# mahbodnr/ViT-CIFAR

Hardware: NVIDIA B200
Metric: train images/s (fwd+bwd+Adam) (higher is better)
Workload: dtype bf16

## Files before the change

### include/vitb200.h

```cpp
#ifndef VITB200_H_
#define VITB200_H_

#include <stddef.h>
#include <stdint.h>

#ifdef __cplusplus
extern "C" {
#endif

#define VITB_F32 0
#define VITB_BF16 1

#define VITB_ABI_VERSION 1

int vitb_version(void);
const char* vitb_last_error(void);
unsigned long long vitb_launch_count(void);
int vitb_device_supported(void);

int vitb_set_l2_persisting_window(void* base, size_t bytes, size_t carve_out_bytes);

int vitb_cast_f32_to_bf16(const float* src, void* dst, int64_t n, void* stream);

size_t vitb_patch_embed_fwd_ws_bytes(int B, int S, int P, int H, int dt);
// ... 17 lines not shown
#define VITB_GEMM_GELU 1
#define VITB_GEMM_OUT_F32 2
int vitb_gemm_bias_act_fwd(const void* a, const void* w_act, const float* bias, const void* residual,
                           void* c, void* preact, int M, int N, int K, int flags, int dt, void* stream);
int vitb_gemm_dgrad(const void* dy, const void* w_act, const void* z, void* dx, int M, int N, int K,
                    int flags, int dt, void* stream);
#define VITB_GEMM_DY_F32 4
size_t vitb_gemm_wgrad_ws_bytes(int M, int N, int K, int dt);
int vitb_gemm_wgrad_dbias(const void* dy, const void* x, float* dw, float* dbias, void* ws,
                          size_t ws_bytes, int M, int N, int K, int flags, int dt, void* stream);

int vitb_attn_fwd(const void* qkv, void* o, float* lse, float* attn_map, int B, int T, int heads,
                  int d, float scale, int dt, void* stream);
int vitb_attn_bwd(const void* qkv, const void* o, const void* d_o, const float* lse, void* dqkv, int B,
                  int T, int heads, int d, float scale, int dt, void* stream);

size_t vitb_colsum_ws_bytes(int rows, int cols);
int vitb_gelu_bwd_colsum(const void* dy, const void* z, void* dz, float* colsum, void* ws,
                         size_t ws_bytes, int rows, int cols, int dt, void* stream);
int vitb_colsum(const void* x, float* colsum, void* ws, size_t ws_bytes, int rows, int cols, int dt,
                void* stream);

int vitb_augment_crop_flip_normalize(const uint8_t* img_u8, const int32_t* dx, const int32_t* dy, const uint8_t* flip,
                                     const float* mean3, const float* std3, float* out, int B, int S, int pad, void* stream);

int vitb_augment_autoaugment(const uint8_t* img_u8, const int32_t* dx, const int32_t* dy, const uint8_t* flip, const int32_t* code,
                             const int32_t* op_ids, const double* mags, int n_sub, const float* mean3, const float* std3,
                             float* out, int B, int S, int pad, void* stream);

int vitb_augment_crop_flip_normalize_gather(const uint8_t* data_u8, const int64_t* labels_src, int N, const int32_t* idx,
// ... 82 lines not shown
```

### vit-cifar_b200/_lib.py

```python
from __future__ import annotations

import ctypes as C
import os
import threading

HERE = os.path.dirname(os.path.abspath(__file__))
LIB_PATH = os.environ.get("VITB_LIB_PATH") or os.path.join(HERE, "libvitb200.so")

F32 = 0
BF16 = 1

GEMM_GELU = 1
GEMM_OUT_F32 = 2
GEMM_DY_F32 = 4

ABI_VERSION = 1

_p = C.c_void_p
_i = C.c_int
_i64 = C.c_int64
_f = C.c_float
_sz = C.c_size_t

class DropoutDesc(C.Structure):
# ... 10 lines not shown
    "vitb_set_l2_persisting_window": (_i, [_p, _sz, _sz]),
    "vitb_cast_f32_to_bf16": (_i, [_p, _p, _i64, _p]),
    "vitb_patch_embed_fwd_ws_bytes": (_sz, [_i, _i, _i, _i, _i]),
    "vitb_patch_embed_fwd": (_i, [_p, _p, _p, _p, _p, _p, _p, _p, _p, _sz, _i, _i, _i, _i, _i, _i, _p]),
    "vitb_patch_embed_bwd_ws_bytes": (_sz, [_i, _i, _i, _i, _i]),
    "vitb_patch_embed_bwd": (_i, [_p, _p, _p, _p, _p, _p, _p, _p, _sz, _i, _i, _i, _i, _i, _i, _p]),
    "vitb_layernorm_fwd": (_i, [_p, _i64, _p, _p, _p, _p, _p, _i, _i, _f, _i, _p]),
    "vitb_layernorm_bwd_ws_bytes": (_sz, [_i, _i]),
    "vitb_layernorm_bwd": (_i, [_p, _p, _i64, _p, _p, _p, _p, _p, _i64, _p, _p, _p, _p, _sz, _i, _i, _i, _p]),
    "vitb_gemm_bias_act_fwd": (_i, [_p, _p, _p, _p, _p, _p, _i, _i, _i, _i, _i, _p]),
    "vitb_gemm_dgrad": (_i, [_p, _p, _p, _p, _i, _i, _i, _i, _i, _p]),
    "vitb_gemm_wgrad_ws_bytes": (_sz, [_i, _i, _i, _i]),
    "vitb_gemm_wgrad_dbias": (_i, [_p, _p, _p, _p, _p, _sz, _i, _i, _i, _i, _i, _p]),
    "vitb_attn_fwd": (_i, [_p, _p, _p, _p, _i, _i, _i, _i, _f, _i, _p]),
    "vitb_attn_bwd": (_i, [_p, _p, _p, _p, _p, _i, _i, _i, _i, _f, _i, _p]),
    "vitb_colsum_ws_bytes": (_sz, [_i, _i]),
    "vitb_gelu_bwd_colsum": (_i, [_p, _p, _p, _p, _p, _sz, _i, _i, _i, _p]),
    "vitb_colsum": (_i, [_p, _p, _p, _sz, _i, _i, _i, _p]),
    "vitb_pool_fwd": (_i, [_p, _p, _i, _i, _i, _i, _i, _p]),
    "vitb_pool_bwd": (_i, [_p, _p, _i, _i, _i, _i, _i, _p]),
    "vitb_augment_crop_flip_normalize": (_i, [_p, _p, _p, _p, _p, _p, _p, _i, _i, _i, _p]),
    "vitb_augment_autoaugment": (_i, [_p, _p, _p, _p, _p, _p, _p, _i, _p, _p, _p, _i, _i, _i, _p]),
    "vitb_augment_crop_flip_normalize_gather": (_i, [_p, _p, _i, _p, _p, _p, _p, _p, _p, _p, _p, _i, _i, _i, _p]),
    "vitb_augment_autoaugment_gather": (_i, [_p, _p, _i, _p, _p, _p, _p, _p, _p, _p, _i, _p, _p, _p, _p, _i, _i, _i, _p]),
    "vitb_batch_mix": (_i, [_p, _p, _p, _i, _i, _i, _i, C.c_double, _i, _i, _i, _i, _p]),
    "vitb_dropout_threshold": (C.c_uint32, [_f]),
    "vitb_dropout": (_i, [_p, _p, _p, _i64, _f, C.c_uint64, C.c_uint32, C.c_uint32, _p, _i, _p]),
    "vitb_ls_ce_fwd_bwd": (_i, [_p, _p, _p, _p, _i, _i, _f, _f, _p]),
    "vitb_ls_ce_mix_fwd_bwd": (_i, [_p, _p, _p, _f, _p, _p, _p, _i, _i, _f, _f, _p]),
    "vitb_ls_ce_batch_fwd_bwd": (_i, [_p, _p, _p, _f, _p, _p, _p, _p, _i, _i, _f, _f, _p]),
# ... 60 lines not shown
```

### vit-cifar_b200/csrc/attention.cu

```cuda
#include <cuda.h>

#include "common.cuh"
#include "gemm_internal.h"

namespace vitb {

__device__ __forceinline__ void ldsm_x4(uint32_t (&r)[4], const void* p) {
  const uint32_t a = (uint32_t)__cvta_generic_to_shared(p);
  asm volatile("ldmatrix.sync.aligned.m8n8.x4.shared.b16 {%0,%1,%2,%3}, [%4];" : "=r"(r[0]), "=r"(r[1]), "=r"(r[2]), "=r"(r[3]) : "r"(a));
}
__device__ __forceinline__ void ldsm_x4_t(uint32_t (&r)[4], const void* p) {
  const uint32_t a = (uint32_t)__cvta_generic_to_shared(p);
  asm volatile("ldmatrix.sync.aligned.m8n8.x4.trans.shared.b16 {%0,%1,%2,%3}, [%4];" : "=r"(r[0]), "=r"(r[1]), "=r"(r[2]), "=r"(r[3]) : "r"(a));
}
__device__ __forceinline__ void stsm_x4(void* p, uint32_t r0, uint32_t r1, uint32_t r2, uint32_t r3) {
  const uint32_t a = (uint32_t)__cvta_generic_to_shared(p);
  asm volatile("stmatrix.sync.aligned.m8n8.x4.shared.b16 [%0], {%1,%2,%3,%4};" ::"r"(a), "r"(r0), "r"(r1), "r"(r2), "r"(r3) : "memory");
}
__device__ __forceinline__ void mma_bf16(float (&d)[4], const uint32_t (&a)[4], uint32_t b0, uint32_t b1) {
  asm volatile(
      "mma.sync.aligned.m16n8k16.row.col.f32.bf16.bf16.f32 {%0,%1,%2,%3}, {%4,%5,%6,%7}, {%8,%9}, {%0,%1,%2,%3};"
      : "+f"(d[0]), "+f"(d[1]), "+f"(d[2]), "+f"(d[3])
      : "r"(a[0]), "r"(a[1]), "r"(a[2]), "r"(a[3]), "r"(b0), "r"(b1));
}
// ... 410 lines not shown

  stage_rows16<D>(dq, sQ, 16 * warp, lane);
  stage_rows16<D>(dk, sK, 16 * warp, lane);
  stage_rows16<D>(dv, sV, 16 * warp, lane);
  fence_async_smem();
  __syncthreads();
  if (tid == 0) {
    tma_store_3d(&m_dqkv, sQ, h * D, 0, b);
    tma_store_3d(&m_dqkv, sK, Hd + h * D, 0, b);
    tma_store_3d(&m_dqkv, sV, 2 * Hd + h * D, 0, b);
    tma_store_commit();
    tma_store_wait_read();
  }
}

__global__ void __launch_bounds__(128)
    attn_fwd_f32_kernel(const float* __restrict__ qkv, float* __restrict__ o, float* __restrict__ lse, float* __restrict__ attn_map,
                        int T, int heads, int D, float scale) {
  pdl_trigger();
  pdl_wait();
  extern __shared__ __align__(16) uint8_t smem_attn[];
  float* sQ = reinterpret_cast<float*>(smem_attn);
  float* sK = sQ + T * D;
  float* sV = sK + T * D;
  float* sS = sV + T * D;
  const int b = blockIdx.x / heads, h = blockIdx.x % heads, Hd = heads * D;
  const int tid = threadIdx.x, nthr = blockDim.x;
  const float* base = qkv + (int64_t)b * T * 3 * Hd + h * D;
  for (int i = tid; i < T * D; i += nthr) {
    const int r = i / D, c = i % D;
// ... 127 lines not shown
    configured = true;
  }
  const int Hd = heads * D;
  CUtensorMap m_qkv, m_o, m_do, m_dqkv;
  if (head_tile_map<D, NT16>(&m_qkv, qkv, 3 * Hd, T, B)) return -1;
  if (head_tile_map<D, NT16>(&m_o, o, Hd, T, B)) return -1;
  if (head_tile_map<D, NT16>(&m_do, d_o, Hd, T, B)) return -1;
  if (head_tile_map<D, NT16>(&m_dqkv, dqkv, 3 * Hd, T, B)) return -1;
  int per_sm = 1;
  VITB_CUDA_OK(cudaOccupancyMaxActiveBlocksPerMultiprocessor(&per_sm, kern, 32 * NT16, smem));
  VITB_LAUNCH((kern), B * heads, 32 * NT16, smem, st, m_qkv, m_o, m_do, m_dqkv, lse, T, heads, scale, kNumSMs * (per_sm > 0 ? per_sm : 1));
  VITB_LAUNCH_OK();
  return 0;
}

#define VITB_ATTN_DISPATCH(FN, ...)                                                   \
  do {                                                                                \
    const int nt = (T + 15) / 16;                                                     \
    if (d == 32) {                                                                    \
      if (nt <= 1) return FN<32, 1>(__VA_ARGS__);                                     \
      if (nt <= 2) return FN<32, 2>(__VA_ARGS__);                                     \
      if (nt <= 4) return FN<32, 4>(__VA_ARGS__);                                     \
      if (nt <= 5) return FN<32, 5>(__VA_ARGS__);                                     \
      return FN<32, 8>(__VA_ARGS__);                                                  \
    } else {                                                                          \
      if (nt <= 1) return FN<64, 1>(__VA_ARGS__);                                     \
      if (nt <= 2) return FN<64, 2>(__VA_ARGS__);                                     \
      if (nt <= 4) return FN<64, 4>(__VA_ARGS__);                                     \
      if (nt <= 5) return FN<64, 5>(__VA_ARGS__);                                     \
      return FN<64, 8>(__VA_ARGS__);                                                  \
// ... 28 lines not shown
int vitb_attn_bwd(const void* qkv, const void* o, const void* d_o, const float* lse, void* dqkv, int B, int T, int heads, int d, float scale,
                  int dt, void* stream) {
  VITB_REQUIRE(qkv && o && d_o && lse && dqkv, "attn_bwd: null pointer");
  VITB_REQUIRE(B > 0 && T > 0 && T <= 128 && heads > 0 && (d == 32 || d == 64), "attn_bwd: unsupported shape B=%d T=%d heads=%d d=%d (T<=128, d in {32,64})", B, T, heads, d);
  cudaStream_t st = (cudaStream_t)stream;
  if (dt == VITB_BF16) {
    VITB_ATTN_DISPATCH(launch_bwd_bf16, qkv, o, d_o, lse, dqkv, B, T, heads, scale, st);
  }
  const size_t smem = ((size_t)4 * T * d + (size_t)2 * T * T) * sizeof(float);
  if (set_dyn_smem((const void*)attn_bwd_f32_kernel, smem)) return -1;
  VITB_LAUNCH((attn_bwd_f32_kernel), B * heads, 128, smem, st, (const float*)qkv, (const float*)d_o, lse, (float*)dqkv, T, heads, d, scale);
  VITB_LAUNCH_OK();
  return 0;
}

}
```

### vit-cifar_b200/engine.py

```python
from __future__ import annotations

import os
from typing import Dict, Optional, Tuple

import torch

from . import functional as Fn
from . import ops
from .layers import act_dtype
from .optim import adam_hyper, sgd_hyper
from .parallel import allreduce_bucket
from .params import LayerViews
from .vit import ViT


class TrainEngine:
    def __init__(self, model: ViT, batch_size: int, smoothing: float = 0.1, lr: float = 1e-3, betas=(0.9, 0.999),
                 eps: float = 1e-8, weight_decay: float = 5e-5, process_group=None, use_graph: bool = True,
                 overlap_comm: bool = False, mixed_targets: bool = False, optimizer: str = "adam", momentum: Optional[float] = None,
                 metrics: bool = False):
        ops.require_device()
        if optimizer not in ("adam", "sgd"):
            raise NotImplementedError(f"Unknown optimizer: {optimizer}")
        self.optimizer = optimizer
# ... 52 lines not shown
                peers, err = None, ValueError("at most 8 ranks of one node and a flat buffer that is a multiple of 4 elements")
            else:
                peers, err = exchange_peer_pointers(dict(g=self.G, p=self.P, c=self.C if self.C is not self.P else None, flags=flags), self.pg)
            ok = torch.tensor([0 if peers is None else 1], device=self.dev)
            dist.all_reduce(ok, op=dist.ReduceOp.MIN, group=self.pg)
            if int(ok.item()) == 1:
                self._fused_dp = dict(peers, flags_t=flags, sync=sync, rank=dist.get_rank(self.pg))
            else:
                import warnings
                warnings.warn(f"fused data-parallel step unavailable ({err}); using one NCCL all-reduce + the Adam kernel")
                self._dp_mode = mode = "single"

        H, M = model.hidden, model.mlp_hidden
        self.dm = Fn.Dims(B=self.B, T=model.num_tokens, H=H, heads=model.head, M=M, use_mlp=model.encoder_mlp)
        self.dm.check()
        mk = lambda buf, i: LayerViews(L, buf, f"enc.{i}.", H, M, model.encoder_mlp)
        self.lp = [mk(self.P, i) for i in range(model.num_layers)]
        self.lc = [mk(self.C, i) for i in range(model.num_layers)]
        self.lg = [mk(self.G, i) for i in range(model.num_layers)]
        v = L.view
        self.has_cls = model.is_cls_token
        self.stem_p = (v(self.P, "emb.weight"), v(self.P, "emb.bias"),
                       v(self.P, "cls_token").view(-1) if self.has_cls else None, v(self.P, "pos_emb").view(model.num_tokens, H))
        self.stem_g = (v(self.G, "emb.weight"), v(self.G, "emb.bias"),
                       v(self.G, "cls_token").view(-1) if self.has_cls else None, v(self.G, "pos_emb").view(model.num_tokens, H))
        self.head_p = (v(self.P, "fc.0.weight"), v(self.P, "fc.0.bias"), v(self.C, "fc.1.weight"), v(self.P, "fc.1.bias"))
        self.head_g = (v(self.G, "fc.0.weight"), v(self.G, "fc.0.bias"), v(self.G, "fc.1.weight"), v(self.G, "fc.1.bias"))
        self.buckets = model.bucket_bounds()

        S = model.img_size
# ... 43 lines not shown
        self._main_stream = None
        env = os.environ.get("VITB_FLUSH_PER_LAYER")
        self._flush_per_layer = (env != "0") if env is not None else (model.hidden * max(model.hidden, model.mlp_hidden) <= 384 * 1536)
        self._opt_per_layer = self._flush_per_layer and self.world == 1 and os.environ.get("VITB_OPT_PER_LAYER", "1") != "0"
        self._opt_done_from = 0
        if ws_mode >= 1:
            if ws_mode >= 2:
                self._main_stream = torch.cuda.Stream(device=self.dev, priority=-1)
            self._side = Fn.SideStream(torch.cuda.Stream(device=self.dev))

    def _alloc(self, scope: str):
        def alloc(name: str, shape: tuple, dtype: torch.dtype) -> torch.Tensor:
            key = f"{scope}.{name}"
            t = self._bufs.get(key)
            if t is None:
                t = (torch.zeros if name == "dxL" else torch.empty)(shape, dtype=dtype, device=self.dev)
                self._bufs[key] = t
            return t
        return alloc

    def _arena_bytes(self) -> int:
        from . import _lib
        lib, dm, m = _lib.load(), self.dm, self.model
        rows, H, M = dm.rows, dm.H, dm.M
        ln = int(lib.vitb_layernorm_bwd_ws_bytes(rows, H))
        pair = lambda N, K: max(ops.wgrad_ws_bytes(rows, N, K), ops.bwd_fused_ws_bytes(rows, N, K))
        per_layer = pair(H, H) + ops.wgrad_ws_bytes(rows, 3 * H, H) + ln
        if dm.use_mlp:
            per_layer += pair(H, M) + pair(M, H) + ln + int(lib.vitb_colsum_ws_bytes(rows, H))
        per_layer += 8 * 256
        return m.num_layers * per_layer + int(lib.vitb_layernorm_bwd_ws_bytes(self.B, H)) + (1 << 20)

    def activation_bytes(self) -> int:
        return sum(t.numel() * t.element_size() for t in self._bufs.values())

    def _allreduce(self, bucket: Tuple[int, int], last: bool = False) -> None:
        if self.world == 1:
            return
        if self._dp_mode in ("none", "fused"):
            return
        if self.overlap_comm:
            allreduce_bucket(self.G, bucket, self.pg, self._comm_stream)
        elif last:
            allreduce_bucket(self.G, (0, self.n), self.pg, None)

    def _body(self) -> None:
        m, dm = self.model, self.dm
        B, T, H, Cn = self.B, m.num_tokens, m.hidden, m.num_classes
        emb_w, emb_b, cls, pos = self.stem_p
        emb_w_c = self.store.layout.view(self.C, "emb.weight") if self.C is not self.P else None
        x, words = Fn.stem_fwd(self.img, emb_w, emb_w_c, emb_b, cls, pos, m.patch, self.act, self._alloc("stem"))
        saved = []
        for i in range(m.num_layers):
            x, sv = Fn.encoder_fwd(x, self.lc[i], self.lp[i], dm, self._alloc(f"l{i}"), drop=self.drops[i] if self.drops else None)
            saved.append(sv)
        ln_w, ln_b, fc_w_c, fc_b = self.head_p
        self.logits, hsaved = Fn.head_fwd(x, ln_w, ln_b, fc_w_c, fc_b, B, T, H, Cn, m.is_cls_token, self._alloc("head"))
        n_valid_dev = self.hyper_dev.view(torch.int32)[11:12]
        if self.mixed_targets:
            ops.ls_ce(self.logits, self.labels, self.loss, self.dlogits, self.smoothing, 1.0, labels_b=self.labels_b, lam_dev=self.hyper_dev[9:10],
                      n_valid_dev=n_valid_dev, ws=self._ls_ws)
        else:
            ops.ls_ce(self.logits, self.labels, self.loss, self.dlogits, self.smoothing, 1.0, n_valid_dev=n_valid_dev, ws=self._ls_ws)
        if self.metrics:
            ops.eval_metrics(self.logits, self.labels, self._record[:3], self._record_ws, self.smoothing, n_valid_dev=n_valid_dev)
            ops.train_loss_accumulate(self.loss, self._record[3:], self.B, n_valid_dev=n_valid_dev)

        self._opt_done_from = self.n
        self._backward(hsaved, saved, words)
        n = self.n
        if self._fused_dp is not None:
            f = self._fused_dp
# ... 17 lines not shown
        ln_w, ln_b, fc_w_c, fc_b = self.head_p
        if self._main_stream is not None:
            outer = torch.cuda.current_stream()
            self._main_stream.wait_stream(outer)
            with torch.cuda.stream(self._main_stream):
                self._backward_kernels(hsaved, saved, words, B, T, H, Cn, ln_w, fc_w_c)
            outer.wait_stream(self._main_stream)
        else:
            self._backward_kernels(hsaved, saved, words, B, T, H, Cn, ln_w, fc_w_c)

    def _backward_kernels(self, hsaved, saved, words, B, T, H, Cn, ln_w, fc_w_c) -> None:
        m, dm, side = self.model, self.dm, self._side
        if self._defer:
            ops.defer_begin(self._arena)
        g_ln_w, g_ln_b, g_fc_w, g_fc_b = self.head_g
        dx = Fn.head_bwd(self.dlogits, hsaved, ln_w, fc_w_c, g_ln_w, g_ln_b, g_fc_w, g_fc_b, B, T, H, Cn, m.is_cls_token, self.act,
                         self._alloc("headb"), dx_prezeroed=True, side=side)
        self._allreduce(self.buckets[-1])
        done = {}
        fuse_below = (Fn.ln_gelu_fused() and dm.use_mlp and self.act == torch.bfloat16 and (not self.drops or Fn._drop_fused(dm.rows)))
        dz2_in = None
        for i in reversed(range(m.num_layers)):
            if side is not None and (i + 2) in done:
                torch.cuda.current_stream().wait_event(done[i + 2])
            below = None
            if fuse_below and i > 0:
                dz2_b = self._alloc(f"bwd_dz2_{(i - 1) % 3}")("dz2", (dm.rows, dm.H), self.act)
                below = (saved[i - 1][4][6], dz2_b, self.lg[i - 1].b2, self.drops[i - 1] if self.drops else None)
            dx = Fn.encoder_bwd(dx, saved[i], self.lc[i], self.lp[i], self.lg[i], dm, self._bwd_alloc(i),
                                drop=self.drops[i] if self.drops else None, side=side, dz2_in=dz2_in, below=below)
            dz2_in = below[1] if below is not None else None
            if side is not None:
                if self._defer and self._flush_per_layer:
                    side.run(ops.defer_flush_partial)
                    if self._opt_per_layer:
                        lo = self.buckets[1 + i][0]
                        hi = self._opt_done_from
                        side.run(lambda lo=lo, hi=hi: self._optimizer_slice(lo, hi))
                        self._opt_done_from = lo
                done[i] = side.done_event()
            self._allreduce(self.buckets[1 + i])
        g_emb_w, g_emb_b, g_cls, g_pos = self.stem_g
        Fn.stem_bwd(self.img, words, dx, g_emb_w, g_emb_b, g_cls, g_pos, m.patch)
        if side is not None:
            side.join()
# ... 182 lines not shown
```

### vit-cifar_b200/functional.py

```python
from __future__ import annotations

import os
from dataclasses import dataclass
from typing import Callable, Optional

import torch

from . import ops
from .params import LayerViews

Alloc = Callable[[str, tuple, torch.dtype], torch.Tensor]


def default_alloc(device: torch.device) -> Alloc:
    def alloc(name: str, shape: tuple, dtype: torch.dtype) -> torch.Tensor:
        return torch.empty(shape, dtype=dtype, device=device)
    return alloc


@dataclass
class Dims:
    B: int
    T: int
    H: int
# ... 70 lines not shown
        return ops.drop_desc(self.p, self.seed, site, self.step, self.step_dev)


DROP_FUSED_MIN_ROWS = 16384


def _drop_fused(rows: int = 1 << 30) -> bool:
    v = os.environ.get("VITB_DROP_FUSED", "auto")
    if v in ("0", "1"):
        return v == "1"
    return rows >= DROP_FUSED_MIN_ROWS


def ln_gelu_fused() -> bool:
    return os.environ.get("VITB_LN_GELU_FUSED", "0") != "0"


def mhsa_fwd(x: torch.Tensor, c: LayerViews, p: LayerViews, dm: Dims, alloc: Alloc, residual: Optional[torch.Tensor],
             attn_map: Optional[torch.Tensor] = None, drop: Optional[Drop] = None):
    rows, H, act = dm.rows, dm.H, x.dtype
    qkv = alloc("qkv", (rows, 3 * H), act)
    ops.gemm_fwd(x, c.wqkv, p.bqkv, None, qkv, None, rows, 3 * H, H)
    o = alloc("o", (rows, H), act)
    lse = alloc("lse", (dm.B, dm.heads, dm.T), torch.float32)
    ops.attn_fwd(qkv, o, lse, attn_map, dm.B, dm.T, dm.heads, dm.d, dm.scale)
    y = alloc("x1", (rows, H), act)
    if drop is None or _drop_fused(rows):
        ops.gemm_fwd(o, c.wo, p.bo, residual, y, None, rows, H, H, drop=drop.desc(0) if drop is not None else None)
    else:
        ops.gemm_fwd(o, c.wo, p.bo, None, y, None, rows, H, H)
# ... 93 lines not shown
            _wgrad(side, dz1, x1n, g.w1, None if b1_done else g.b1, rows, M, H)
            ops.gemm_dgrad(dz1, c.w1, None, dx1n, rows, M, H)
        dx1 = alloc("dx1", (rows, H), act)
        if fused_drop:
            dya = alloc("dao", (rows, H), act)
            ops.layernorm_bwd_fused(dx1n, x1, H, p.ln2_w, mean2, rstd2, dout, dx1, H, g.ln2_w, g.ln2_b, None, dya, g.bo, rows, H,
                                    drop=drop.desc(0))
            bo_done = True
        else:
            bo_done = drop is None
            ops.layernorm_bwd(dx1n, x1, H, p.ln2_w, mean2, rstd2, dout, dx1, H, g.ln2_w, g.ln2_b, g.bo if bo_done else None, rows, H)
    else:
        dx1 = dout
        bo_done = False
    dxn = mhsa_bwd(dx1, att_saved, c, g, dm, alloc, bo_done=bo_done, drop=drop, side=side, dy_masked=dya)
    dx = alloc("dx", (rows, H), act)
    if below is not None:
        z2_b, dz2_b, g_b2_b, drop_b = below
        ops.layernorm_bwd_fused(dxn, x, H, p.ln1_w, mean1, rstd1, dx1, dx, H, g.ln1_w, g.ln1_b, z2_b, dz2_b, g_b2_b, rows, H,
                                drop=drop_b.desc(2) if drop_b is not None else None)
    else:
        ops.layernorm_bwd(dxn, x, H, p.ln1_w, mean1, rstd1, dx1, dx, H, g.ln1_w, g.ln1_b, None, rows, H)
    return dx


def stem_fwd(img: torch.Tensor, emb_w, emb_w_c, emb_b, cls, pos, P: int, act: torch.dtype, alloc: Alloc):
    B, _, S, _ = img.shape
    has_cls = cls is not None
    T = P * P + (1 if has_cls else 0)
    H, K = emb_w.shape
    x0 = alloc("x0", (B * T, H), act)
    words = alloc("words", (B * P * P, K), act) if (act == torch.bfloat16 and emb_w_c is not None) else None
    ops.patch_embed_fwd(img, emb_w, emb_w_c if words is not None else None, emb_b, cls, pos, x0, words, P, has_cls)
    return x0, words


def stem_bwd(img: torch.Tensor, words, dx0: torch.Tensor, g_emb_w, g_emb_b, g_cls, g_pos, P: int) -> None:
    ops.patch_embed_bwd(img, words, dx0, g_emb_w, g_emb_b, g_cls, g_pos, P, g_cls is not None)
# ... 34 lines not shown
```

### vit-cifar_b200/ops.py

```python
from __future__ import annotations

import ctypes as C
from typing import Optional

import torch

from . import _lib
from ._lib import BF16, F32, GEMM_DY_F32, GEMM_GELU, GEMM_OUT_F32, check

_DT = {torch.float32: F32, torch.bfloat16: BF16}


def dt_of(t: torch.Tensor) -> int:
    try:
        return _DT[t.dtype]
    except KeyError:
        raise TypeError(f"activation dtype must be float32 or bfloat16, got {t.dtype}") from None


def _ptr(t: Optional[torch.Tensor]) -> Optional[int]:
    if t is None:
        return None
    if not t.is_cuda:
        raise _lib.VitbError("libvitb200 kernels take CUDA tensors only (no CPU fallback)")
# ... 134 lines not shown
    lib = _lib.load()
    dt = dt_of(x)
    nb = lib.vitb_gemm_bwd_fused_ws_bytes(M, N, K, dt)
    ws = workspace(max(int(nb), 256), x.device)
    check(lib.vitb_gemm_bwd_fused(_ptr(dy), _ptr(x), _ptr(w_act), _ptr(z), _ptr(dx), _ptr(dw), _ptr(dx_colsum), _ptr(ws), ws.numel(), M, N, K, dt,
                                  _stream()), "gemm_bwd_fused")


def attn_fwd(qkv, o, lse, attn_map, B: int, T: int, heads: int, d: int, scale: float) -> None:
    check(_lib.load().vitb_attn_fwd(_ptr(qkv), _ptr(o), _ptr(lse), _ptr(attn_map), B, T, heads, d, scale, dt_of(qkv), _stream()), "attn_fwd")


def attn_bwd(qkv, o, d_o, lse, dqkv, B: int, T: int, heads: int, d: int, scale: float) -> None:
    check(_lib.load().vitb_attn_bwd(_ptr(qkv), _ptr(o), _ptr(d_o), _ptr(lse), _ptr(dqkv), B, T, heads, d, scale, dt_of(qkv), _stream()),
          "attn_bwd")


def gelu_bwd_colsum(dy, z, dz, colsum, rows: int, cols: int, drop=None) -> None:
    lib = _lib.load()
    ws = workspace(lib.vitb_colsum_ws_bytes(rows, cols), dy.device)
    check(lib.vitb_gelu_bwd_colsum_drop(_ptr(dy), _ptr(z), _ptr(dz), _ptr(colsum), _ptr(ws), ws.numel(), rows, cols, dt_of(dy), _dref(drop),
                                        _stream()), "gelu_bwd_colsum")


def colsum(x, out, rows: int, cols: int) -> None:
    lib = _lib.load()
    ws = workspace(lib.vitb_colsum_ws_bytes(rows, cols), x.device)
    check(lib.vitb_colsum(_ptr(x), _ptr(out), _ptr(ws), ws.numel(), rows, cols, dt_of(x), _stream()), "colsum")


# ... 249 lines not shown
```

Baseline: 171,700.

## Compute only the CLS token in the last encoder layer

When the model classifies from the CLS token, the last encoder layer now computes attention only for the CLS query, and runs the output projection and MLP only on B rows instead of B*T rows. New single-warp forward and backward attention kernels handle the one-query case, and the backward scatters the CLS residual gradient back into a zeroed full-row buffer. This removes the per-token work in the last layer whose outputs the head never reads. In exchange it adds new kernels and a separate code path that is used only for bf16, zero dropout and batch size of at least 32.

```diff
diff --git a/include/vitb200.h b/include/vitb200.h
--- a/include/vitb200.h
+++ b/include/vitb200.h
@@ -55,6 +55,10 @@
                   int d, float scale, int dt, void* stream);
 int vitb_attn_bwd(const void* qkv, const void* o, const void* d_o, const float* lse, void* dqkv, int B,
                   int T, int heads, int d, float scale, int dt, void* stream);
+int vitb_attn_cls_fwd(const void* qkv, void* o_c, float* lse_c, int B, int T, int heads, int d, float scale, int dt,
+                      void* stream);
+int vitb_attn_cls_bwd(const void* qkv, const void* o_c, const void* do_c, const float* lse_c, void* dqkv, int B, int T,
+                      int heads, int d, float scale, int dt, void* stream);
 
 size_t vitb_colsum_ws_bytes(int rows, int cols);
 int vitb_gelu_bwd_colsum(const void* dy, const void* z, void* dz, float* colsum, void* ws,
diff --git a/vit-cifar_b200/_lib.py b/vit-cifar_b200/_lib.py
--- a/vit-cifar_b200/_lib.py
+++ b/vit-cifar_b200/_lib.py
@@ -48,6 +48,8 @@
     "vitb_gemm_wgrad_dbias": (_i, [_p, _p, _p, _p, _p, _sz, _i, _i, _i, _i, _i, _p]),
     "vitb_attn_fwd": (_i, [_p, _p, _p, _p, _i, _i, _i, _i, _f, _i, _p]),
     "vitb_attn_bwd": (_i, [_p, _p, _p, _p, _p, _i, _i, _i, _i, _f, _i, _p]),
+    "vitb_attn_cls_fwd": (_i, [_p, _p, _p, _i, _i, _i, _i, _f, _i, _p]),
+    "vitb_attn_cls_bwd": (_i, [_p, _p, _p, _p, _p, _i, _i, _i, _i, _f, _i, _p]),
     "vitb_colsum_ws_bytes": (_sz, [_i, _i]),
     "vitb_gelu_bwd_colsum": (_i, [_p, _p, _p, _p, _p, _sz, _i, _i, _i, _p]),
     "vitb_colsum": (_i, [_p, _p, _p, _sz, _i, _i, _i, _p]),
diff --git a/vit-cifar_b200/csrc/attention.cu b/vit-cifar_b200/csrc/attention.cu
--- a/vit-cifar_b200/csrc/attention.cu
+++ b/vit-cifar_b200/csrc/attention.cu
@@ -448,6 +448,233 @@
   }
 }
 
+template <int D, int NT16>
+__global__ void __launch_bounds__(32)
+    attn_cls_fwd_bf16_kernel(const __grid_constant__ CUtensorMap m_q, const __grid_constant__ CUtensorMap m_qkv, bf16* __restrict__ o,
+                             float* __restrict__ lse, int T, int heads, float scale, int pf_dist) {
+  constexpr int TP = 16 * NT16;
+  constexpr uint32_t TILE_B = TP * D * 2, ROWS_B = 16 * D * 2;
+  extern __shared__ uint8_t smem_attn_raw[];
+  const uint32_t sbase = (smem_u32(smem_attn_raw) + 1023u) & ~1023u;
+  const uint32_t sQ = sbase, sK = sQ + ROWS_B, sV = sK + TILE_B, bar = sV + TILE_B;
+  const int b = blockIdx.x / heads, h = blockIdx.x % heads, Hd = heads * D;
+  const int lane = threadIdx.x;
+  pdl_trigger();
+  if (lane == 0) {
+    mbar_init(bar, 1);
+    asm volatile("fence.mbarrier_init.release.cluster;" ::: "memory");
+  }
+  __syncthreads();
+  pdl_wait();
+  if (lane == 0) {
+    mbar_arrive_expect_tx(bar, ROWS_B + 2 * TILE_B);
+    tma_load_3d(sQ, &m_q, bar, h * D, 0, b);
+    tma_load_3d(sK, &m_qkv, bar, Hd + h * D, 0, b);
+    tma_load_3d(sV, &m_qkv, bar, 2 * Hd + h * D, 0, b);
+    const int nxt = (int)blockIdx.x + pf_dist;
+    if (nxt < (int)gridDim.x) {
+      const int nb = nxt / heads, nh = nxt % heads;
+      tma_prefetch_3d(&m_qkv, Hd + nh * D, 0, nb);
+      tma_prefetch_3d(&m_qkv, 2 * Hd + nh * D, 0, nb);
+    }
+  }
+  const int g = lane >> 2, t = lane & 3;
+  const float sl2 = scale * kLog2e;
+  const KeyMask km = make_key_mask(T, lane);
+  const LaneAddr<D> la(lane);
+  mbar_wait(bar, 0);
+
+  float s[2 * NT16][4];
+  qk_tile<D, NT16>(s, sQ, sK, 0, la, km);
+  float m0 = -INFINITY, m1 = -INFINITY;
+#pragma unroll
+  for (int j = 0; j < 2 * NT16; ++j) {
+    m0 = fmaxf(m0, fmaxf(s[j][0], s[j][1]));
+    m1 = fmaxf(m1, fmaxf(s[j][2], s[j][3]));
+  }
+  m0 = quad_max(m0);
+  m1 = quad_max(m1);
+  const float ms0 = m0 * sl2, ms1 = m1 * sl2;
+  float sum0 = 0.f, sum1 = 0.f;
+#pragma unroll
+  for (int j = 0; j < 2 * NT16; ++j) {
+    s[j][0] = ex2_fast(fmaf(s[j][0], sl2, -ms0));
+    s[j][1] = ex2_fast(fmaf(s[j][1], sl2, -ms0));
+    s[j][2] = ex2_fast(fmaf(s[j][2], sl2, -ms1));
+    s[j][3] = ex2_fast(fmaf(s[j][3], sl2, -ms1));
+    sum0 += s[j][0] + s[j][1];
+    sum1 += s[j][2] + s[j][3];
+  }
+  sum0 = quad_sum(sum0);
+  const float inv0 = 1.0f / sum0;
+  float acc[D / 8][4];
+#pragma unroll
+  for (int jn = 0; jn < D / 8; ++jn) acc[jn][0] = acc[jn][1] = acc[jn][2] = acc[jn][3] = 0.f;
+  pv_tile<D, NT16>(acc, s, sV, la);
+  if (g == 0) {
+    if (t == 0) lse[(int64_t)b * heads + h] = m0 * scale + logf(sum0);
+    bf16* orow = o + (int64_t)b * Hd + h * D;
+#pragma unroll
+    for (int jn = 0; jn < D / 8; ++jn)
+      *reinterpret_cast<uint32_t*>(orow + 8 * jn + 2 * t) = pack_bf16x2(acc[jn][0] * inv0, acc[jn][1] * inv0);
+  }
+}
+
+template <int D, int NT16>
+__global__ void __launch_bounds__(32)
+    attn_cls_bwd_bf16_kernel(const __grid_constant__ CUtensorMap m_q, const __grid_constant__ CUtensorMap m_qkv, const __grid_constant__ CUtensorMap m_o,
+                             const __grid_constant__ CUtensorMap m_do, const __grid_constant__ CUtensorMap m_dqkv, const float* __restrict__ lse,
+                             int T, int heads, float scale, int pf_dist) {
+  constexpr int TP = 16 * NT16, LP = TP + 8, CH = D / 8;
+  constexpr uint32_t TILE_B = TP * D * 2, ROWS_B = 16 * D * 2;
+  extern __shared__ uint8_t smem_attn_raw[];
+  const uint32_t sbase = (smem_u32(smem_attn_raw) + 1023u) & ~1023u;
+  uint8_t* gen = smem_attn_raw + (sbase - smem_u32(smem_attn_raw));
+  const uint32_t sQ = sbase, sK = sQ + TILE_B, sV = sK + TILE_B, sdO = sV + TILE_B, sO = sdO + ROWS_B;
+  bf16* sP = reinterpret_cast<bf16*>(gen + 3 * TILE_B + 2 * ROWS_B);
+  bf16* sdS = sP + 16 * LP;
+  float* sD = reinterpret_cast<float*>(sdS + 16 * LP);
+  const uint32_t bar = smem_u32(sD + 16);
+  const int b = blockIdx.x / heads, h = blockIdx.x % heads, Hd = heads * D;
+  const int lane = threadIdx.x;
+  pdl_trigger();
+  pdl_wait();
+  if (lane == 0) {
+    mbar_init(bar, 1);
+    asm volatile("fence.mbarrier_init.release.cluster;" ::: "memory");
+    mbar_arrive_expect_tx(bar, 3 * TILE_B + 2 * ROWS_B);
+    tma_load_3d(sQ, &m_q, bar, h * D, 0, b);
+    tma_load_3d(sK, &m_qkv, bar, Hd + h * D, 0, b);
+    tma_load_3d(sV, &m_qkv, bar, 2 * Hd + h * D, 0, b);
+    tma_load_3d(sdO, &m_do, bar, h * D, 0, b);
+    tma_load_3d(sO, &m_o, bar, h * D, 0, b);
+    const int nxt = (int)blockIdx.x + pf_dist;
+    if (nxt < (int)gridDim.x) {
+      const int nb = nxt / heads, nh = nxt % heads;
+      tma_prefetch_3d(&m_qkv, Hd + nh * D, 0, nb);
+      tma_prefetch_3d(&m_qkv, 2 * Hd + nh * D, 0, nb);
+    }
+  }
+  const int g = lane >> 2;
+  const float l0 = g == 0 ? lse[(int64_t)b * heads + h] * kLog2e : 0.f, l1 = 0.f;
+  __syncthreads();
+  mbar_wait(bar, 0);
+  for (int idx = lane; idx < 16 * CH; idx += 32) {
+    const int r = idx / CH, c = idx % CH;
+    uint32_t a0, a1, a2, a3, q0, q1, q2, q3;
+    const uint32_t off = tile_off<D>(r, c);
+    asm volatile("ld.shared.v4.b32 {%0, %1, %2, %3}, [%4];" : "=r"(a0), "=r"(a1), "=r"(a2), "=r"(a3) : "r"(sdO + off));
+    asm volatile("ld.shared.v4.b32 {%0, %1, %2, %3}, [%4];" : "=r"(q0), "=r"(q1), "=r"(q2), "=r"(q3) : "r"(sO + off));
+    const float2 x0 = unpack_bf16x2(a0), x1 = unpack_bf16x2(a1), x2 = unpack_bf16x2(a2), x3 = unpack_bf16x2(a3);
+    const float2 y0 = unpack_bf16x2(q0), y1 = unpack_bf16x2(q1), y2 = unpack_bf16x2(q2), y3 = unpack_bf16x2(q3);
+    float v = (x0.x * y0.x + x0.y * y0.y) + (x1.x * y1.x + x1.y * y1.y) + (x2.x * y2.x + x2.y * y2.y) + (x3.x * y3.x + x3.y * y3.y);
+#pragma unroll
+    for (int off2 = CH / 2; off2 > 0; off2 >>= 1) v += __shfl_xor_sync(0xffffffffu, v, off2);
+    if (c == 0) sD[r] = v;
+  }
+  __syncwarp();
+
+  const float sl2 = scale * kLog2e;
+  const float d0 = sD[g], d1 = sD[g + 8];
+  const KeyMask km = make_key_mask(T, lane);
+  const LaneAddr<D> la(lane);
+  uint32_t aq[D / 16][4], ado[D / 16][4];
+#pragma unroll
+  for (int kk = 0; kk < D / 16; ++kk) {
+    ldsm_x4_s(aq[kk], sQ + la.a(0, kk));
+    ldsm_x4_s(ado[kk], sdO + la.a(0, kk));
+  }
+  float dq[D / 8][4];
+#pragma unroll
+  for (int jn = 0; jn < D / 8; ++jn) dq[jn][0] = dq[jn][1] = dq[jn][2] = dq[jn][3] = 0.f;
+#pragma unroll
+  for (int jc = 0; jc < NT16; ++jc) {
+    float s[2][4], dp[2][4];
+#pragma unroll
+    for (int u = 0; u < 2; ++u) {
+      const int j = 2 * jc + u;
+      s[u][0] = s[u][1] = s[u][2] = s[u][3] = 0.f;
+      dp[u][0] = dp[u][1] = dp[u][2] = dp[u][3] = 0.f;
+      if (j < km.nfull || (j == km.nfull && km.rem != 0)) {
+#pragma unroll
+        for (int k2 = 0; k2 < D / 32; ++k2) {
+          uint32_t bk[4], bv[4];
+          ldsm_x4_s(bk, sK + la.b(8 * j, k2));
+          ldsm_x4_s(bv, sV + la.b(8 * j, k2));
+          mma_bf16(s[u], aq[2 * k2], bk[0], bk[1]);
+          mma_bf16(s[u], aq[2 * k2 + 1], bk[2], bk[3]);
+          mma_bf16(dp[u], ado[2 * k2], bv[0], bv[1]);
+          mma_bf16(dp[u], ado[2 * k2 + 1], bv[2], bv[3]);
+        }
+        if (j == km.nfull) {
+          s[u][0] += km.pm0; s[u][2] += km.pm0;
+          s[u][1] += km.pm1; s[u][3] += km.pm1;
+        }
+        s[u][0] = ex2_fast(fmaf(s[u][0], sl2, -l0));
+        s[u][1] = ex2_fast(fmaf(s[u][1], sl2, -l0));
+        s[u][2] = ex2_fast(fmaf(s[u][2], sl2, -l1));
+        s[u][3] = ex2_fast(fmaf(s[u][3], sl2, -l1));
+        dp[u][0] = s[u][0] * (dp[u][0] - d0) * scale;
+        dp[u][1] = s[u][1] * (dp[u][1] - d0) * scale;
+        dp[u][2] = s[u][2] * (dp[u][2] - d1) * scale;
+        dp[u][3] = s[u][3] * (dp[u][3] - d1) * scale;
+      }
+    }
+    uint32_t pa[4], da[4];
+    pa[0] = pack_bf16x2(s[0][0], s[0][1]); pa[1] = pack_bf16x2(s[0][2], s[0][3]);
+    pa[2] = pack_bf16x2(s[1][0], s[1][1]); pa[3] = pack_bf16x2(s[1][2], s[1][3]);
+    da[0] = pack_bf16x2(dp[0][0], dp[0][1]); da[1] = pack_bf16x2(dp[0][2], dp[0][3]);
+    da[2] = pack_bf16x2(dp[1][0], dp[1][1]); da[3] = pack_bf16x2(dp[1][2], dp[1][3]);
+    const int srow = ((lane >> 3) & 1) * 8 + (lane & 7), scol = 16 * jc + (lane >> 4) * 8;
+    stsm_x4(sP + srow * LP + scol, pa[0], pa[1], pa[2], pa[3]);
+    stsm_x4(sdS + srow * LP + scol, da[0], da[1], da[2], da[3]);
+#pragma unroll
+    for (int jp = 0; jp < D / 16; ++jp) {
+      uint32_t bb[4];
+      ldsm_x4_t_s(bb, sK + la.t(16 * jc, jp));
+      mma_bf16(dq[2 * jp], da, bb[0], bb[1]);
+      mma_bf16(dq[2 * jp + 1], da, bb[2], bb[3]);
+    }
+  }
+  __syncwarp();
+
+  for (int kt = 0; kt < NT16; ++kt) {
+    float dv[D / 8][4], dk[D / 8][4];
+#pragma unroll
+    for (int jn = 0; jn < D / 8; ++jn) {
+      dv[jn][0] = dv[jn][1] = dv[jn][2] = dv[jn][3] = 0.f;
+      dk[jn][0] = dk[jn][1] = dk[jn][2] = dk[jn][3] = 0.f;
+    }
+    const int arow = ((lane & 7) + ((lane >> 4) & 1) * 8) * LP + 16 * kt + ((lane >> 3) & 1) * 8;
+    uint32_t ap[4], as[4];
+    ldsm_x4_t(ap, sP + arow);
+    ldsm_x4_t(as, sdS + arow);
+#pragma unroll
+    for (int jp = 0; jp < D / 16; ++jp) {
+      uint32_t bo[4], bq[4];
+      ldsm_x4_t_s(bo, sdO + la.t(0, jp));
+      ldsm_x4_t_s(bq, sQ + la.t(0, jp));
+      mma_bf16(dv[2 * jp], ap, bo[0], bo[1]);
+      mma_bf16(dv[2 * jp + 1], ap, bo[2], bo[3]);
+      mma_bf16(dk[2 * jp], as, bq[0], bq[1]);
+      mma_bf16(dk[2 * jp + 1], as, bq[2], bq[3]);
+    }
+    stage_rows16<D>(dk, sK, 16 * kt, lane);
+    stage_rows16<D>(dv, sV, 16 * kt, lane);
+  }
+  __syncwarp();
+  stage_rows16<D>(dq, sQ, 0, lane);
+  fence_async_smem();
+  __syncwarp();
+  if (lane == 0) {
+    tma_store_3d(&m_dqkv, sQ, h * D, 0, b);
+    tma_store_3d(&m_dqkv, sK, Hd + h * D, 0, b);
+    tma_store_3d(&m_dqkv, sV, 2 * Hd + h * D, 0, b);
+    tma_store_commit();
+    tma_store_wait_read();
+  }
+}
+
 __global__ void __launch_bounds__(128)
     attn_fwd_f32_kernel(const float* __restrict__ qkv, float* __restrict__ o, float* __restrict__ lse, float* __restrict__ attn_map,
                         int T, int heads, int D, float scale) {
@@ -605,6 +832,55 @@
   return 0;
 }
 
+template <int D>
+static int row0_map(CUtensorMap* map, const void* ptr, int cols, int T, int B, int box_rows) {
+  return make_tma_map_3d_bf16(map, ptr, (uint64_t)cols, 1, (uint64_t)B, (uint64_t)cols * 2, (uint64_t)T * cols * 2, D, box_rows, 1, D == 32 ? 64 : 128);
+}
+
+template <int D, int NT16>
+static int launch_cls_fwd_bf16(const void* qkv, void* o, float* lse, int B, int T, int heads, float scale, cudaStream_t st) {
+  constexpr int TP = 16 * NT16;
+  constexpr size_t smem = (size_t)16 * D * 2 + (size_t)2 * TP * D * 2 + 16 + 1024;
+  auto kern = attn_cls_fwd_bf16_kernel<D, NT16>;
+  static int per_sm = 0;
+  if (per_sm == 0) {
+    VITB_CUDA_OK(cudaFuncSetAttribute(kern, cudaFuncAttributeMaxDynamicSharedMemorySize, (int)smem));
+    VITB_CUDA_OK(cudaOccupancyMaxActiveBlocksPerMultiprocessor(&per_sm, kern, 32, smem));
+    if (per_sm < 1) per_sm = 1;
+  }
+  const int Hd = heads * D;
+  CUtensorMap m_q, m_qkv;
+  if (row0_map<D>(&m_q, qkv, 3 * Hd, T, B, 16)) return -1;
+  if (head_tile_map<D, NT16>(&m_qkv, qkv, 3 * Hd, T, B)) return -1;
+  VITB_LAUNCH((kern), B * heads, 32, smem, st, m_q, m_qkv, (bf16*)o, lse, T, heads, scale, kNumSMs * per_sm);
+  VITB_LAUNCH_OK();
+  return 0;
+}
+
+template <int D, int NT16>
+static int launch_cls_bwd_bf16(const void* qkv, const void* o, const void* d_o, const float* lse, void* dqkv, int B, int T, int heads, float scale,
+                               cudaStream_t st) {
+  constexpr int TP = 16 * NT16, LP = TP + 8;
+  constexpr size_t smem = (size_t)3 * TP * D * 2 + (size_t)2 * 16 * D * 2 + (size_t)2 * 16 * LP * 2 + 16 * sizeof(float) + 16 + 1024;
+  auto kern = attn_cls_bwd_bf16_kernel<D, NT16>;
+  static int per_sm = 0;
+  if (per_sm == 0) {
+    VITB_CUDA_OK(cudaFuncSetAttribute(kern, cudaFuncAttributeMaxDynamicSharedMemorySize, (int)smem));
+    VITB_CUDA_OK(cudaOccupancyMaxActiveBlocksPerMultiprocessor(&per_sm, kern, 32, smem));
+    if (per_sm < 1) per_sm = 1;
+  }
+  const int Hd = heads * D;
+  CUtensorMap m_q, m_qkv, m_o, m_do, m_dqkv;
+  if (row0_map<D>(&m_q, qkv, 3 * Hd, T, B, TP)) return -1;
+  if (head_tile_map<D, NT16>(&m_qkv, qkv, 3 * Hd, T, B)) return -1;
+  if (row0_map<D>(&m_o, o, Hd, 1, B, 16)) return -1;
+  if (row0_map<D>(&m_do, d_o, Hd, 1, B, 16)) return -1;
+  if (head_tile_map<D, NT16>(&m_dqkv, dqkv, 3 * Hd, T, B)) return -1;
+  VITB_LAUNCH((kern), B * heads, 32, smem, st, m_q, m_qkv, m_o, m_do, m_dqkv, lse, T, heads, scale, kNumSMs * per_sm);
+  VITB_LAUNCH_OK();
+  return 0;
+}
+
 #define VITB_ATTN_DISPATCH(FN, ...)                                                   \
   do {                                                                                \
     const int nt = (T + 15) / 16;                                                     \
@@ -663,4 +939,21 @@
   return 0;
 }
 
-}
+int vitb_attn_cls_fwd(const void* qkv, void* o_c, float* lse_c, int B, int T, int heads, int d, float scale, int dt, void* stream) {
+  VITB_REQUIRE(qkv && o_c && lse_c, "attn_cls_fwd: null pointer");
+  VITB_REQUIRE(dt == VITB_BF16, "attn_cls_fwd: bf16 only (dt=%d)", dt);
+  VITB_REQUIRE(B > 0 && T > 0 && T <= 128 && heads > 0 && (d == 32 || d == 64), "attn_cls_fwd: unsupported shape B=%d T=%d heads=%d d=%d (T<=128, d in {32,64})", B, T, heads, d);
+  cudaStream_t st = (cudaStream_t)stream;
+  VITB_ATTN_DISPATCH(launch_cls_fwd_bf16, qkv, o_c, lse_c, B, T, heads, scale, st);
+}
+
+int vitb_attn_cls_bwd(const void* qkv, const void* o_c, const void* do_c, const float* lse_c, void* dqkv, int B, int T, int heads, int d,
+                      float scale, int dt, void* stream) {
+  VITB_REQUIRE(qkv && o_c && do_c && lse_c && dqkv, "attn_cls_bwd: null pointer");
+  VITB_REQUIRE(dt == VITB_BF16, "attn_cls_bwd: bf16 only (dt=%d)", dt);
+  VITB_REQUIRE(B > 0 && T > 0 && T <= 128 && heads > 0 && (d == 32 || d == 64), "attn_cls_bwd: unsupported shape B=%d T=%d heads=%d d=%d (T<=128, d in {32,64})", B, T, heads, d);
+  cudaStream_t st = (cudaStream_t)stream;
+  VITB_ATTN_DISPATCH(launch_cls_bwd_bf16, qkv, o_c, do_c, lse_c, dqkv, B, T, heads, scale, st);
+}
+
+}
diff --git a/vit-cifar_b200/engine.py b/vit-cifar_b200/engine.py
--- a/vit-cifar_b200/engine.py
+++ b/vit-cifar_b200/engine.py
@@ -90,6 +90,8 @@
         H, M = model.hidden, model.mlp_hidden
         self.dm = Fn.Dims(B=self.B, T=model.num_tokens, H=H, heads=model.head, M=M, use_mlp=model.encoder_mlp)
         self.dm.check()
+        self._cls_tail = Fn.cls_tail(model.is_cls_token, self.act, model.p_drop, self.B)
+        self._head_T = 1 if self._cls_tail else model.num_tokens
         mk = lambda buf, i: LayerViews(L, buf, f"enc.{i}.", H, M, model.encoder_mlp)
         self.lp = [mk(self.P, i) for i in range(model.num_layers)]
         self.lc = [mk(self.C, i) for i in range(model.num_layers)]
@@ -163,7 +165,7 @@
             key = f"{scope}.{name}"
             t = self._bufs.get(key)
             if t is None:
-                t = (torch.zeros if name == "dxL" else torch.empty)(shape, dtype=dtype, device=self.dev)
+                t = (torch.zeros if name in ("dxL", "dx1_rows") else torch.empty)(shape, dtype=dtype, device=self.dev)
                 self._bufs[key] = t
             return t
         return alloc
@@ -172,13 +174,16 @@
         from . import _lib
         lib, dm, m = _lib.load(), self.dm, self.model
         rows, H, M = dm.rows, dm.H, dm.M
-        ln = int(lib.vitb_layernorm_bwd_ws_bytes(rows, H))
-        pair = lambda N, K: max(ops.wgrad_ws_bytes(rows, N, K), ops.bwd_fused_ws_bytes(rows, N, K))
-        per_layer = pair(H, H) + ops.wgrad_ws_bytes(rows, 3 * H, H) + ln
-        if dm.use_mlp:
-            per_layer += pair(H, M) + pair(M, H) + ln + int(lib.vitb_colsum_ws_bytes(rows, H))
-        per_layer += 8 * 256
-        return m.num_layers * per_layer + int(lib.vitb_layernorm_bwd_ws_bytes(self.B, H)) + (1 << 20)
+        ln = lambda r: int(lib.vitb_layernorm_bwd_ws_bytes(r, H))
+        pair = lambda r, N, K: max(ops.wgrad_ws_bytes(r, N, K), ops.bwd_fused_ws_bytes(r, N, K))
+
+        def per_layer(r: int) -> int:
+            n = pair(r, H, H) + ops.wgrad_ws_bytes(rows, 3 * H, H) + ln(rows)
+            if dm.use_mlp:
+                n += pair(r, H, M) + pair(r, M, H) + ln(r) + int(lib.vitb_colsum_ws_bytes(r, H))
+            return n + 8 * 256
+        last = per_layer(self.B if self._cls_tail else rows)
+        return (m.num_layers - 1) * per_layer(rows) + last + ln(self.B) + (1 << 20)
 
     def activation_bytes(self) -> int:
         return sum(t.numel() * t.element_size() for t in self._bufs.values())
@@ -201,10 +206,13 @@
         x, words = Fn.stem_fwd(self.img, emb_w, emb_w_c, emb_b, cls, pos, m.patch, self.act, self._alloc("stem"))
         saved = []
         for i in range(m.num_layers):
-            x, sv = Fn.encoder_fwd(x, self.lc[i], self.lp[i], dm, self._alloc(f"l{i}"), drop=self.drops[i] if self.drops else None)
+            if self._cls_tail and i == m.num_layers - 1:
+                x, sv = Fn.encoder_cls_fwd(x, self.lc[i], self.lp[i], dm, self._alloc(f"l{i}"))
+            else:
+                x, sv = Fn.encoder_fwd(x, self.lc[i], self.lp[i], dm, self._alloc(f"l{i}"), drop=self.drops[i] if self.drops else None)
             saved.append(sv)
         ln_w, ln_b, fc_w_c, fc_b = self.head_p
-        self.logits, hsaved = Fn.head_fwd(x, ln_w, ln_b, fc_w_c, fc_b, B, T, H, Cn, m.is_cls_token, self._alloc("head"))
+        self.logits, hsaved = Fn.head_fwd(x, ln_w, ln_b, fc_w_c, fc_b, B, self._head_T, H, Cn, m.is_cls_token, self._alloc("head"))
         n_valid_dev = self.hyper_dev.view(torch.int32)[11:12]
         if self.mixed_targets:
             ops.ls_ce(self.logits, self.labels, self.loss, self.dlogits, self.smoothing, 1.0, labels_b=self.labels_b, lam_dev=self.hyper_dev[9:10],
@@ -252,7 +260,7 @@
         if self._defer:
             ops.defer_begin(self._arena)
         g_ln_w, g_ln_b, g_fc_w, g_fc_b = self.head_g
-        dx = Fn.head_bwd(self.dlogits, hsaved, ln_w, fc_w_c, g_ln_w, g_ln_b, g_fc_w, g_fc_b, B, T, H, Cn, m.is_cls_token, self.act,
+        dx = Fn.head_bwd(self.dlogits, hsaved, ln_w, fc_w_c, g_ln_w, g_ln_b, g_fc_w, g_fc_b, B, self._head_T, H, Cn, m.is_cls_token, self.act,
                          self._alloc("headb"), dx_prezeroed=True, side=side)
         self._allreduce(self.buckets[-1])
         done = {}
@@ -265,8 +273,11 @@
             if fuse_below and i > 0:
                 dz2_b = self._alloc(f"bwd_dz2_{(i - 1) % 3}")("dz2", (dm.rows, dm.H), self.act)
                 below = (saved[i - 1][4][6], dz2_b, self.lg[i - 1].b2, self.drops[i - 1] if self.drops else None)
-            dx = Fn.encoder_bwd(dx, saved[i], self.lc[i], self.lp[i], self.lg[i], dm, self._bwd_alloc(i),
-                                drop=self.drops[i] if self.drops else None, side=side, dz2_in=dz2_in, below=below)
+            if self._cls_tail and i == m.num_layers - 1:
+                dx = Fn.encoder_cls_bwd(dx, saved[i], self.lc[i], self.lp[i], self.lg[i], dm, self._bwd_alloc(i), side=side, below=below)
+            else:
+                dx = Fn.encoder_bwd(dx, saved[i], self.lc[i], self.lp[i], self.lg[i], dm, self._bwd_alloc(i),
+                                    drop=self.drops[i] if self.drops else None, side=side, dz2_in=dz2_in, below=below)
             dz2_in = below[1] if below is not None else None
             if side is not None:
                 if self._defer and self._flush_per_layer:
diff --git a/vit-cifar_b200/functional.py b/vit-cifar_b200/functional.py
--- a/vit-cifar_b200/functional.py
+++ b/vit-cifar_b200/functional.py
@@ -108,6 +108,15 @@
 
 def ln_gelu_fused() -> bool:
     return os.environ.get("VITB_LN_GELU_FUSED", "0") != "0"
+
+
+CLS_TAIL_MIN_B = 32
+
+
+def cls_tail(is_cls: bool, act: torch.dtype, p_drop: float, B: int) -> bool:
+    if os.environ.get("VITB_CLS_TAIL", "auto") == "0":
+        return False
+    return bool(is_cls) and act == torch.bfloat16 and p_drop == 0.0 and B >= CLS_TAIL_MIN_B
 
 
 def mhsa_fwd(x: torch.Tensor, c: LayerViews, p: LayerViews, dm: Dims, alloc: Alloc, residual: Optional[torch.Tensor],
@@ -231,14 +240,82 @@
         dx1 = dout
         bo_done = False
     dxn = mhsa_bwd(dx1, att_saved, c, g, dm, alloc, bo_done=bo_done, drop=drop, side=side, dy_masked=dya)
-    dx = alloc("dx", (rows, H), act)
+    return _ln1_bwd(dxn, x, mean1, rstd1, dx1, p, g, dm, alloc, below)
+
+
+def _ln1_bwd(dxn, x, mean1, rstd1, dres, p: LayerViews, g: LayerViews, dm: Dims, alloc: Alloc, below: Optional[tuple]) -> torch.Tensor:
+    rows, H = dm.rows, dm.H
+    dx = alloc("dx", (rows, H), dxn.dtype)
     if below is not None:
         z2_b, dz2_b, g_b2_b, drop_b = below
-        ops.layernorm_bwd_fused(dxn, x, H, p.ln1_w, mean1, rstd1, dx1, dx, H, g.ln1_w, g.ln1_b, z2_b, dz2_b, g_b2_b, rows, H,
+        ops.layernorm_bwd_fused(dxn, x, H, p.ln1_w, mean1, rstd1, dres, dx, H, g.ln1_w, g.ln1_b, z2_b, dz2_b, g_b2_b, rows, H,
                                 drop=drop_b.desc(2) if drop_b is not None else None)
     else:
-        ops.layernorm_bwd(dxn, x, H, p.ln1_w, mean1, rstd1, dx1, dx, H, g.ln1_w, g.ln1_b, None, rows, H)
+        ops.layernorm_bwd(dxn, x, H, p.ln1_w, mean1, rstd1, dres, dx, H, g.ln1_w, g.ln1_b, None, rows, H)
     return dx
+
+
+def encoder_cls_fwd(x: torch.Tensor, c: LayerViews, p: LayerViews, dm: Dims, alloc: Alloc):
+    B, rows, H, M, act = dm.B, dm.rows, dm.H, dm.M, x.dtype
+    xn = alloc("xn", (rows, H), act)
+    mean1 = alloc("mean1", (rows,), torch.float32)
+    rstd1 = alloc("rstd1", (rows,), torch.float32)
+    ops.layernorm_fwd(x, H, p.ln1_w, p.ln1_b, xn, mean1, rstd1, rows, H)
+    qkv = alloc("qkv", (rows, 3 * H), act)
+    ops.gemm_fwd(xn, c.wqkv, p.bqkv, None, qkv, None, rows, 3 * H, H)
+    o_c = alloc("o_c", (B, H), act)
+    lse_c = alloc("lse_c", (B, dm.heads), torch.float32)
+    ops.attn_cls_fwd(qkv, o_c, lse_c, B, dm.T, dm.heads, dm.d, dm.scale)
+    x_c = alloc("x_c", (B, H), act)
+    ops.pool_fwd(x, x_c, B, dm.T, H, 0)
+    x1 = alloc("x1_c", (B, H), act)
+    ops.gemm_fwd(o_c, c.wo, p.bo, x_c, x1, None, B, H, H)
+    att_saved = (xn, qkv, o_c, lse_c)
+    if not dm.use_mlp:
+        return x1, (x, mean1, rstd1, att_saved, None)
+    x1n = alloc("x1n_c", (B, H), act)
+    mean2 = alloc("mean2_c", (B,), torch.float32)
+    rstd2 = alloc("rstd2_c", (B,), torch.float32)
+    ops.layernorm_fwd(x1, H, p.ln2_w, p.ln2_b, x1n, mean2, rstd2, B, H)
+    z1 = alloc("z1_c", (B, M), act)
+    a1 = alloc("a1_c", (B, M), act)
+    z2 = alloc("z2_c", (B, H), act)
+    x2 = alloc("x2_c", (B, H), act)
+    ops.gemm_fwd(x1n, c.w1, p.b1, None, a1, z1, B, M, H, gelu=True)
+    ops.gemm_fwd(a1, c.w2, p.b2, x1, x2, z2, B, H, M, gelu=True)
+    return x2, (x, mean1, rstd1, att_saved, (x1, x1n, mean2, rstd2, z1, a1, z2))
+
+
+def encoder_cls_bwd(dout_c: torch.Tensor, saved, c: LayerViews, p: LayerViews, g: LayerViews, dm: Dims, alloc: Alloc,
+                    side: Optional[SideStream] = None, below: Optional[tuple] = None) -> torch.Tensor:
+    x, mean1, rstd1, (xn, qkv, o_c, lse_c), mlp_saved = saved
+    B, rows, H, M, act = dm.B, dm.rows, dm.H, dm.M, dout_c.dtype
+    if dm.use_mlp:
+        x1, x1n, mean2, rstd2, z1, a1, z2 = mlp_saved
+        dz2 = alloc("dz2_c", (B, H), act)
+        ops.gelu_bwd_colsum(dout_c, z2, dz2, g.b2, B, H)
+        _wgrad(side, dz2, a1, g.w2, None, B, H, M)
+        dz1 = alloc("dz1_c", (B, M), act)
+        ops.gemm_dgrad(dz2, c.w2, z1, dz1, B, H, M)
+        _wgrad(side, dz1, x1n, g.w1, g.b1, B, M, H)
+        dx1n = alloc("dx1n_c", (B, H), act)
+        ops.gemm_dgrad(dz1, c.w1, None, dx1n, B, M, H)
+        dx1 = alloc("dx1_c", (B, H), act)
+        ops.layernorm_bwd(dx1n, x1, H, p.ln2_w, mean2, rstd2, dout_c, dx1, H, g.ln2_w, g.ln2_b, g.bo, B, H)
+        bo_done = True
+    else:
+        dx1, bo_done = dout_c, False
+    _wgrad(side, dx1, o_c, g.wo, None if bo_done else g.bo, B, H, H)
+    do_c = alloc("do_c", (B, H), act)
+    ops.gemm_dgrad(dx1, c.wo, None, do_c, B, H, H)
+    dqkv = alloc("dqkv", (rows, 3 * H), act)
+    ops.attn_cls_bwd(qkv, o_c, do_c, lse_c, dqkv, B, dm.T, dm.heads, dm.d, dm.scale)
+    _wgrad(side, dqkv, xn, g.wqkv, g.bqkv, rows, 3 * H, H)
+    dxn = alloc("dxn", (rows, H), act)
+    ops.gemm_dgrad(dqkv, c.wqkv, None, dxn, rows, 3 * H, H)
+    dres = alloc("dx1_rows", (rows, H), act)
+    ops.pool_bwd(dx1, dres, B, dm.T, H, 2)
+    return _ln1_bwd(dxn, x, mean1, rstd1, dres, p, g, dm, alloc, below)
 
 
 def stem_fwd(img: torch.Tensor, emb_w, emb_w_c, emb_b, cls, pos, P: int, act: torch.dtype, alloc: Alloc):
diff --git a/vit-cifar_b200/ops.py b/vit-cifar_b200/ops.py
--- a/vit-cifar_b200/ops.py
+++ b/vit-cifar_b200/ops.py
@@ -172,6 +172,32 @@
 def attn_bwd(qkv, o, d_o, lse, dqkv, B: int, T: int, heads: int, d: int, scale: float) -> None:
     check(_lib.load().vitb_attn_bwd(_ptr(qkv), _ptr(o), _ptr(d_o), _ptr(lse), _ptr(dqkv), B, T, heads, d, scale, dt_of(qkv), _stream()),
           "attn_bwd")
+
+
+def _check_cls_attn(B: int, T: int, heads: int, d: int, **ts) -> None:
+    H = heads * d
+    want = {"qkv": ((B * T, 3 * H), torch.bfloat16), "dqkv": ((B * T, 3 * H), torch.bfloat16), "o_c": ((B, H), torch.bfloat16),
+            "do_c": ((B, H), torch.bfloat16), "lse_c": ((B, heads), torch.float32)}
+    for name, t in ts.items():
+        shape, dt = want[name]
+        if t.dtype != dt or t.numel() != shape[0] * shape[1]:
+            raise ValueError(f"attn_cls: {name} must be {dt} with {shape[0]} x {shape[1]} elements, got {t.dtype} {tuple(t.shape)}")
+    dev = ts["qkv"].device
+    for name, t in ts.items():
+        if not t.is_cuda or t.device != dev:
+            raise ValueError(f"attn_cls: every operand must be on the same CUDA device ({name} is on {t.device}, qkv on {dev})")
+    _contig(*ts.values())
+
+
+def attn_cls_fwd(qkv, o_c, lse_c, B: int, T: int, heads: int, d: int, scale: float) -> None:
+    _check_cls_attn(B, T, heads, d, qkv=qkv, o_c=o_c, lse_c=lse_c)
+    check(_lib.load().vitb_attn_cls_fwd(_ptr(qkv), _ptr(o_c), _ptr(lse_c), B, T, heads, d, scale, BF16, _stream()), "attn_cls_fwd")
+
+
+def attn_cls_bwd(qkv, o_c, do_c, lse_c, dqkv, B: int, T: int, heads: int, d: int, scale: float) -> None:
+    _check_cls_attn(B, T, heads, d, qkv=qkv, o_c=o_c, do_c=do_c, lse_c=lse_c, dqkv=dqkv)
+    check(_lib.load().vitb_attn_cls_bwd(_ptr(qkv), _ptr(o_c), _ptr(do_c), _ptr(lse_c), _ptr(dqkv), B, T, heads, d, scale, BF16, _stream()),
+          "attn_cls_bwd")
 
 
 def gelu_bwd_colsum(dy, z, dz, colsum, rows: int, cols: int, drop=None) -> None:
```

New measurement: 184,500 (median of 6 runs). +7.4%, better.
